# martellab-sri/ModalTune

Hardware: AMD Instinct MI355X
Metric: slides/sec (train step) at 10k patches x 1536-d (higher is better)
Workload: dtype f16; 1 GPU; Prov-GigaPath ModalAdapter train step, 10000 patches x 1536-d, 6 pathways -> 64 gene tokens + 1 task token, 3 task passes, fp16 operands / fp32 accumulate, 1 slide per GPU per step, task passes as two concurrent groups (B = 2 | 1 on two HIP streams), train mode: Dropout(0.25) on the embedded input and both backbone branches, DropPath(0..0.1) per layer and on the Extractor FFN (Philox masks regener; patches=10000, parallelism=dp1, dropout=True

## Files before the change

include/modaltune_hip.h:

```cpp
#ifndef MODALTUNE_HIP_H
#define MODALTUNE_HIP_H

#include <stdint.h>

#ifdef __cplusplus
extern "C" {
#endif

typedef void* mt_stream_t;
typedef uint16_t mt_half;

typedef enum {
  MT_OK = 0,
  MT_ERR_BAD_ARG = -1,
  MT_ERR_LAUNCH = -2,
  MT_ERR_UNSUPPORTED = -3
} MtStatus;

typedef struct { int seg_rows, seg_stride, row0; } MtRowMap;

typedef struct {
  float eps;
  const int* live;
  int live_rows;
  float* partials;
  long partials_elems;
  int grid_wgs;
} MtLaunchOpts;

int mt_version(void);
const char* mt_status_string(int status);
const char* mt_build_id(void);

enum { MT_EPI_BIAS = 0,
       MT_EPI_BIAS_RESID = 1,
       MT_EPI_INJECT = 2,
       MT_EPI_POSEMB = 3,
       MT_EPI_QKV_HM = 4 };
enum { MT_OUT_F16 = 0, MT_OUT_F32 = 1 };

typedef struct {
  const unsigned* rng;
  unsigned site;
  float p;
  unsigned path_site;
  float path_p;
  int rows_per_pass;
} MtDropout;
int mt_rng_advance(unsigned* rng, mt_stream_t stream);
int mt_dropout_f32(const float* x, long ldx, const MtRowMap* xmap, float* y, int M, int D, const MtDropout* drop,
                   mt_stream_t stream);
int mt_droppath_rows_f32(float* x, int M, int D, const MtDropout* drop, mt_stream_t stream);

#define MT_LIVE_SITES_MAX 64
int mt_droppath_live(const unsigned* path_sites, const float* path_ps, int n, int B, const unsigned* rng, int* table,
                     mt_stream_t stream);

typedef struct {
  const float* bias;
  const float* resid;
  long ldr;
  MtRowMap rmap;
  const float* colscale;
  const float* pos_table;
  const int* pos_row;
  const int* pos_col;
  MtDropout drop;
} MtGemmEpilogue;

int mt_gemm_nt_f16(const mt_half* A, long lda, const MtRowMap* amap, const mt_half* W, int M, int N, int K,
                   int epilogue, const MtGemmEpilogue* epi, void* C, long ldc, const MtRowMap* cmap, int out_dtype,
                   const MtLaunchOpts* opt, mt_stream_t stream);

int mt_gemm_tn_f16(const mt_half* A, long lda, const MtRowMap* amap, const mt_half* B, long ldb, const MtRowMap* bmap,
                   int M, int N1, int N2, float* C, long ldc, float* colsum, const MtLaunchOpts* opt, mt_stream_t stream);

int mt_colsum_f16(const mt_half* A, long lda, const MtRowMap* amap, int M, int N, float* out, const MtLaunchOpts* opt,
                  mt_stream_t stream);

enum { MT_ACT_NONE = 0, MT_ACT_RELU = 1, MT_ACT_GELU = 2, MT_ACT_ELU = 3 };
// ... 249 lines not shown
```

modaltune_amd/_lib.py:

```python
from __future__ import annotations

import ctypes as C
import os

_HERE = os.path.dirname(os.path.abspath(__file__))
LIB_PATH = os.environ.get("MODALTUNE_HIP_LIB", os.path.join(_HERE, "_C", "libmodaltune_hip.so"))

P, I, L, F, D = C.c_void_p, C.c_int, C.c_long, C.c_float, C.c_double


class MtRowMap(C.Structure):
    _fields_ = [("seg_rows", I), ("seg_stride", I), ("row0", I)]


class MtDropout(C.Structure):
    _fields_ = [("rng", P), ("site", C.c_uint), ("p", F), ("path_site", C.c_uint), ("path_p", F), ("rows_per_pass", I)]


class MtGemmEpilogue(C.Structure):
    _fields_ = [("bias", P), ("resid", P), ("ldr", L), ("rmap", MtRowMap), ("colscale", P),
                ("pos_table", P), ("pos_row", P), ("pos_col", P), ("drop", MtDropout)]


class MtLaunchOpts(C.Structure):
    _fields_ = [("eps", F), ("live", P), ("live_rows", I), ("partials", P), ("partials_elems", L), ("grid_wgs", I)]


MT_SGEMM_MAX = 3


class MtSgemm(C.Structure):
    _fields_ = [("A", P), ("as0", L), ("as1", L), ("a_bs", L), ("B", P), ("bs0", L), ("bs1", L), ("b_bs", L),
                ("bias", P), ("bias_on_m", I), ("C", P), ("cs0", L), ("cs1", L), ("c_bs", L),
                ("M", I), ("N", I), ("K", I), ("batch", I), ("act", I), ("accumulate", I),
                ("rowsum", P), ("pre_out", P), ("resid", P), ("c_drop", MtDropout),
                ("a_aux", P), ("a_act", I), ("a_drop", MtDropout), ("resid_scale", F), ("a_ld", I)]


MT_MAX_BRANCHES = 8


class MtDilatedPlan(C.Structure):
    _fields_ = [("nbranch", I), ("N", I), ("B", I), ("seg", I * MT_MAX_BRANCHES), ("ratio", I * MT_MAX_BRANCHES),
                ("nseg", I * MT_MAX_BRANCHES), ("n", I * MT_MAX_BRANCHES), ("qlimit", I * MT_MAX_BRANCHES)]


class MtDensePlan(C.Structure):
    _fields_ = [("N", I), ("B", I), ("H", I), ("dist", P), ("nslope", P)]


class MtLongNetLayerWeights(C.Structure):
    _fields_ = [(n, P) for n in ("ln1_w", "ln1_b", "inner_ln_w", "inner_ln_b", "ln2_w", "ln2_b", "ffn_ln_w", "ffn_ln_b", "b_qkv", "b_out",
                                 "b_fc1", "b_fc2", "w_qkv", "w_out", "w_fc1", "w_fc2", "wt_qkv", "wt_out", "wt_fc1", "wt_fc2")]


class MtLongNetLayerBuffers(C.Structure):
    _fields_ = [(n, P) for n in ("hin", "hmid", "qkv", "o_br", "lse_br", "lse_tot", "a1", "st1", "stin", "st2", "stf", "u16", "br16", "t16",
                                 "dh", "dy16", "dh16", "dt16", "da1", "dmixed", "dqkv16", "delta", "attn_ws", "live_attn", "live_ffn")]


class MtVitBlockWeights(C.Structure):
    _fields_ = [(n, P) for n in ("n1_w", "n1_b", "n2_w", "n2_b")] + [("n1_eps", F), ("n2_eps", F)] + \
               [(n, P) for n in ("b_qkv", "b_proj", "b_fc1", "b_fc2", "w_qkv", "w_proj", "w_fc1", "w_fc2", "wt_qkv", "wt_proj", "wt_fc1", "wt_fc2")]


class MtVitBlockBuffers(C.Structure):
    _fields_ = [(n, P) for n in ("hin", "hmid", "qkv", "o16", "lse", "a1", "st1", "st2", "u16", "br16", "t16", "dh", "dy16", "dh16", "dt16",
                                 "da1", "dqkv16", "delta")]


RM = C.POINTER(MtRowMap)
DR = C.POINTER(MtDropout)
EP = C.POINTER(MtGemmEpilogue)
PL = C.POINTER(MtDilatedPlan)
DP = C.POINTER(MtDensePlan)
OP = C.POINTER(MtLaunchOpts)

SIGNATURES = {
# ... 139 lines not shown
```

modaltune_amd/csrc/attn.hip:

```cpp
#include "attn_common.h"

namespace {

template <bool LIVE>
__global__ __launch_bounds__(256) void dilated_attn_fwd_kernel(const h16* __restrict__ qkv, Plan p, h16* __restrict__ o_br,
                                                               float* __restrict__ lse_br) {
  __shared__ __attribute__((aligned(16))) h16 smem[4 * IMG_HALVES];
  h16* const Ks = smem;
  h16* const Vs = smem + 2 * IMG_HALVES;
  const int tid = threadIdx.x, lane = tid & 63, wave = tid >> 6;
  const int hh = lane >> 5, l31 = lane & 31;
  const WorkItem w = decode(p, blockIdx.x);
  const Seq sq = make_seq(p, w);
  const long M = (long)p.B * p.N;
  const int nv = __builtin_amdgcn_readfirstlane(sq.nvalid());
  const int nvq = min(nv, p.qlimit[w.br]);
  if (w.qt * 128 >= nvq || (LIVE && pass_dead(p, w.b))) return;

  {
    const int buf = tid >> 7, row = (tid >> 1) & 63, which = 6 + (tid & 1);
    const h16x8 one = {(h16)1.f, 0, 0, 0, (h16)1.f, 0, 0, 0}, zero = {0, 0, 0, 0, 0, 0, 0, 0};
    *reinterpret_cast<h16x8*>(&Vs[buf * IMG_HALVES + img_off(row, which)]) = which == 6 ? one : zero;
  }

  const int iq = w.qt * 128 + wave * 32 + l31;
  const bool qvalid = sq.valid(iq) && iq < nvq;
  const long qrow = sq.row_clamped(iq);
  h16x8 qf[3];
#pragma unroll
  for (int ks = 0; ks < 3; ++ks)
    qf[ks] = sel8(qvalid, ldg8(hm_ptr(qkv, M, w.h, qrow) + ks * 16 + hh * 8));

  const int ntile = (sq.n + 63) / 64;
  const int nproc = (nv + 63) >> 6;
  const int row_bytes = sq.dr * HD * 2;
  const long valid_bytes = (long)(nv - 1) * row_bytes + HD * 2;
  const long tile_bytes = 64L * row_bytes;
  const h16* const kseq = hm_ptr(qkv, M, H + w.h, sq.row(0));
  const h16* const vseq = hm_ptr(qkv, M, 2 * H + w.h, sq.row(0));
  const DmaLane dl(tid, row_bytes);
  auto dma = [&](int t) {
    dma_tile(Ks + (t & 1) * IMG_HALVES, tile_rsrc(kseq, t * tile_bytes, valid_bytes), dl);
    dma_tile(Vs + (t & 1) * IMG_HALVES, tile_rsrc(vseq, t * tile_bytes, valid_bytes), dl);
  };
  const int grp = lane >> 4, li = lane & 15, tq = li >> 2, tp = li & 3;
  int krd[3];
#pragma unroll
  for (int ks = 0; ks < 3; ++ks) krd[ks] = img_off(l31, 2 * ks + hh);
  const int vc = 2 * (grp & 1) + (tp >> 1), vo = 4 * (tp & 1);
  const int va0 = img_off(4 * hh + tq, vc) + vo, va1 = img_off(4 * hh + tq, vc + 4) + vo;
  const int vb0 = img_off(4 * hh + tq + 8, vc) + vo, vb1 = img_off(4 * hh + tq + 8, vc + 4) + vo;

  auto qk = [&](const h16* Kb, f32x16 (&s)[2], const f32x16& init) {
#pragma unroll
    for (int sub = 0; sub < 2; ++sub) {
#pragma unroll
      for (int ks = 0; ks < 3; ++ks) {
        const h16x8 kf = *reinterpret_cast<const h16x8*>(&Kb[sub * 32 * IMG_ROW + krd[ks]]);
        s[sub] = __builtin_amdgcn_mfma_f32_32x32x16_f16(kf, qf[ks], ks == 0 ? init : s[sub], 0, 0, 0);
      }
    }
  };

  f32x16 o0, o1;
#pragma unroll
  for (int i = 0; i < 16; ++i) { o0[i] = 0.f; o1[i] = 0.f; }

  dma(0);
  dma_wait_all();
  __syncthreads();
  float m2;
  f32x16 minit;
  {
    f32x16 s0[2], zero;
#pragma unroll
    for (int i = 0; i < 16; ++i) zero[i] = 0.f;
    qk(Ks, s0, zero);
    float mx = NEG_BIG;
#pragma unroll
    for (int sub = 0; sub < 2; ++sub)
#pragma unroll
      for (int i = 0; i < 16; ++i) {
        const int kidx = sub * 32 + (i & 3) + 8 * (i >> 2) + 4 * hh;
        mx = fmaxf(mx, kidx < sq.n ? s0[sub][i] : NEG_BIG);
      }
    m2 = max_halves(mx);
#pragma unroll
    for (int i = 0; i < 16; ++i) minit[i] = -m2;
  }

  auto tile = [&](int t, auto tail_tag) {
    constexpr bool TAIL = decltype(tail_tag)::value;
    const int kb = t * 64;
    const h16* Kb = Ks + (t & 1) * IMG_HALVES;
    const h16* Vb = Vs + (t & 1) * IMG_HALVES;
    if (t + 1 < nproc) dma(t + 1);
    f32x16 s_cur[2];
    qk(Kb, s_cur, minit);
    float mx = NEG_BIG;
#pragma unroll
    for (int sub = 0; sub < 2; ++sub)
#pragma unroll
      for (int i = 0; i < 16; ++i) {
        if (TAIL) {
          const int kidx = kb + sub * 32 + (i & 3) + 8 * (i >> 2) + 4 * hh;
          if (kidx >= sq.n) s_cur[sub][i] = NEG_BIG;
        }
        mx = fmaxf(mx, s_cur[sub][i]);
      }
    mx = max_halves(mx);
    if (__any(mx > RESCALE_LOG2)) {
      const float up = fmaxf(mx, 0.f);
      const float alpha = __builtin_amdgcn_exp2f(-up);
#pragma unroll
      for (int i = 0; i < 16; ++i) { o0[i] *= alpha; o1[i] *= alpha; s_cur[0][i] -= up; s_cur[1][i] -= up; }
      m2 += up;
#pragma unroll
      for (int i = 0; i < 16; ++i) minit[i] = -m2;
    }
#pragma unroll
    for (int sub = 0; sub < 2; ++sub)
#pragma unroll
      for (int s2 = 0; s2 < 2; ++s2) {
        h16x8 pf;
#pragma unroll
        for (int e = 0; e < 8; e += 2) {
          const f32x2 a = pk_exp2((f32x2){s_cur[sub][8 * s2 + e], s_cur[sub][8 * s2 + e + 1]});
          pf[e] = (h16)a[0]; pf[e + 1] = (h16)a[1];
        }
        const h16* vblk = Vb + (sub * 32 + s2 * 16) * IMG_ROW;
        const h16x8 v0 = cat8(lds_tr4(vblk + va0), lds_tr4(vblk + vb0));
        const h16x8 v1 = cat8(lds_tr4(vblk + va1), lds_tr4(vblk + vb1));
        o0 = __builtin_amdgcn_mfma_f32_32x32x16_f16(v0, pf, o0, 0, 0, 0);
        o1 = __builtin_amdgcn_mfma_f32_32x32x16_f16(v1, pf, o1, 0, 0, 0);
      }
    dma_wait_all();
    __syncthreads();
  };
  const bool tail_last = nproc == ntile && (sq.n & 63);
  const int nplain = tail_last ? nproc - 1 : nproc;
  for (int t = 0; t < nplain; ++t) tile(t, std::false_type{});
  if (tail_last) tile(nproc - 1, std::true_type{});
  const int rest = sq.n - nproc * 64;
  if (rest > 0) {
    if (__any(-m2 > RESCALE_LOG2)) {
      const float up = fmaxf(-m2, 0.f);
      const float alpha = __builtin_amdgcn_exp2f(-up);
#pragma unroll
      for (int i = 0; i < 16; ++i) { o0[i] *= alpha; o1[i] *= alpha; }
      m2 += up;
    }
    o1[8] += (float)rest * __builtin_amdgcn_exp2f(-m2);
  }

  if (qvalid) {
    const float l = o1[8];
    const float inv = 1.0f / l;
    h16* orow = o_br + ((long)w.br * M + qrow) * DM + w.h * HD;
#pragma unroll
    for (int gq = 0; gq < 4; ++gq) {
      h16x4 v = {(h16)(o0[4 * gq] * inv), (h16)(o0[4 * gq + 1] * inv), (h16)(o0[4 * gq + 2] * inv), (h16)(o0[4 * gq + 3] * inv)};
      *reinterpret_cast<h16x4*>(orow + 8 * gq + 4 * hh) = v;
    }
#pragma unroll
    for (int gq = 0; gq < 2; ++gq) {
      h16x4 v = {(h16)(o1[4 * gq] * inv), (h16)(o1[4 * gq + 1] * inv), (h16)(o1[4 * gq + 2] * inv), (h16)(o1[4 * gq + 3] * inv)};
      *reinterpret_cast<h16x4*>(orow + 32 + 8 * gq + 4 * hh) = v;
    }
    if (hh == 0) lse_br[((long)w.br * M + qrow) * H + w.h] = (m2 + __log2f(l)) * LN2;
  }
}

struct MixGeom {
  int grp[MT_MAX_BRANCHES];
  MT_DEVINL MixGeom(const Plan& p, int h) {
#pragma unroll
    for (int b = 0; b < MT_MAX_BRANCHES; ++b) grp[b] = b < p.nbranch ? h / (H / p.ratio[b]) : -1;
  }
};
MT_DEVINL void seg_split(const Plan& p, int b, int pos, int& j, int& loc) {
  const int sg = p.seg[b];
  if (sg >= p.N) { j = 0; loc = pos; return; }
  j = (int)((float)pos * p.inv_seg[b]);
  loc = pos - j * sg;
  if (loc < 0) { loc += sg; --j; }
  if (loc >= sg) { loc -= sg; ++j; }
}
MT_DEVINL int residue(const Plan& p, int b, int pos) {
  int j, loc;
  seg_split(p, b, pos, j, loc);
  const int dr = p.ratio[b];
  return (dr & (dr - 1)) == 0 ? (loc & (dr - 1)) : loc % dr;
}
MT_DEVINL int dense_branch(const Plan& p) {
  int d = 0;
#pragma unroll
  for (int b = 0; b < MT_MAX_BRANCHES; ++b) if (b < p.nbranch && p.ratio[b] == 1) d = b;
  return d;
}
constexpr int MIX_CPL = 24;
struct H24 { h16x8 a, b, c; };
MT_DEVINL H24 ld24(const h16* p) {
  return H24{*reinterpret_cast<const h16x8*>(p), *reinterpret_cast<const h16x8*>(p + 8), *reinterpret_cast<const h16x8*>(p + 16)};
}
MT_DEVINL float h24(const H24& v, int e) { return (float)(e < 8 ? v.a[e & 7] : e < 16 ? v.b[e & 7] : v.c[e & 7]); }
MT_DEVINL float half_sum(float v) {
// ... 98 lines not shown
    for (int b = 0; b < NB; ++b) {
      cov[b] = b < p.nbranch && geo.grp[b] == residue(p, b, pos);
      const int sb = cov[b] ? b : db;
      lse[b] = lse_br[((long)sb * M + m) * H + h];
      ob[b] = ld24(o_br + ((long)sb * M + m) * DM + c0);
    }
    float v[MIX_CPL];
#pragma unroll
    for (int e = 0; e < MIX_CPL; ++e) v[e] = 0.f;
#pragma unroll
    for (int b = 0; b < NB; ++b) {
      const float wgt = cov[b] ? __expf(lse[b] - tot) : 0.f;
#pragma unroll
      for (int e = 0; e < MIX_CPL; ++e) v[e] = fmaf(wgt, cov[b] ? h24(ob[b], e) : 0.f, v[e]);
    }
    float g[MIX_CPL], xh[MIX_CPL];
    float s1 = 0.f, s2 = 0.f;
#pragma unroll
    for (int i = 0; i < MIX_CPL; ++i) {
      xh[i] = (v[i] - mean) * rstd;
      g[i] = h24(dyv, i) * w[i];
      s1 += g[i]; s2 = fmaf(g[i], xh[i], s2);
    }
    const float c1 = half_sum(s1) * (1.0f / DM), c2 = half_sum(s2) * (1.0f / DM);
    float dm[MIX_CPL];
    h16* dst = dmixed + ((long)h * M + m) * HD + (c0 - h * HD);
#pragma unroll
    for (int k = 0; k < 3; ++k) {
      h16x8 o;
#pragma unroll
      for (int e = 0; e < 8; ++e) {
        const int i = 8 * k + e;
        o[e] = (h16)(rstd * (g[i] - c1 - xh[i] * c2));
        dm[i] = (float)o[e];
      }
      if (live) *reinterpret_cast<h16x8*>(dst + 8 * k) = o;
    }
#pragma unroll
    for (int b = 0; b < NB; ++b) {
      float d = 0.f;
#pragma unroll
      for (int e = 0; e < MIX_CPL; ++e) d = fmaf(dm[e], h24(ob[b], e), d);
      d += __shfl_xor(d, 1, 64);
      if (live && (l5 & 1) == 0 && cov[b]) delta_br[((long)b * M + m) * H + h] = d;
    }
  }
}


}

extern "C" int mt_dilated_attn_fwd(const mt_half* qkv, const MtDilatedPlan* plan, mt_half* o_br, float* lse_br, const MtLaunchOpts* opt,
                                   mt_stream_t stream) {
  if (int rc = mt_opts_check(opt, MT_OPT_LIVE)) return rc;
  if (!qkv || !o_br || !lse_br || !plan_ok(plan)) return MT_ERR_BAD_ARG;
  const Plan p = make_plan(plan, 128, mt_opt_live(opt));
  const int nblk = p.blk_off[p.nbranch];
  if (p.live) hipLaunchKernelGGL(dilated_attn_fwd_kernel<true>, dim3(nblk), dim3(256), 0, (hipStream_t)stream, (const h16*)qkv, p,
                     (h16*)o_br, lse_br);
  else hipLaunchKernelGGL(dilated_attn_fwd_kernel<false>, dim3(nblk), dim3(256), 0, (hipStream_t)stream, (const h16*)qkv, p,
                     (h16*)o_br, lse_br);
  MT_CHECK_LAUNCH();
  return MT_OK;
}

constexpr int MIX_CUS = 256, MIX_FWD_WG_PER_CU = 3, MIX_BWD_WG_PER_CU = 2;
static dim3 mix_grid(long M, int grid_wgs, int wg_per_cu) {
  return dim3((int)min((M + 7) / 8, (long)(grid_wgs > 0 ? grid_wgs : wg_per_cu * MIX_CUS)));
}

extern "C" int mt_dilated_mix_ln_fwd(const mt_half* o_br, const float* lse_br, const MtDilatedPlan* plan,
                                     const float* ln_w, const float* ln_b, mt_half* y, float* stats, float* lse_tot,
                                     const MtLaunchOpts* opt, mt_stream_t stream) {
  if (int rc = mt_opts_check(opt, MT_OPT_LIVE | MT_OPT_GRID)) return rc;
  if (!o_br || !lse_br || !ln_w || !ln_b || !y || !stats || !lse_tot || !plan_ok(plan)) return MT_ERR_BAD_ARG;
  const Plan p = make_plan(plan, 128, mt_opt_live(opt));
  const long M = (long)p.B * p.N;
  const dim3 grid = mix_grid(M, opt ? opt->grid_wgs : 0, MIX_FWD_WG_PER_CU);
  if (p.nbranch <= 5)
    hipLaunchKernelGGL(mix_ln_fwd_kernel<5>, grid, dim3(256), 0, (hipStream_t)stream, (const h16*)o_br, lse_br, p, ln_w, ln_b,
                       (h16*)y, stats, lse_tot);
  else
    hipLaunchKernelGGL(mix_ln_fwd_kernel<MT_MAX_BRANCHES>, grid, dim3(256), 0, (hipStream_t)stream, (const h16*)o_br, lse_br, p,
                       ln_w, ln_b, (h16*)y, stats, lse_tot);
  MT_CHECK_LAUNCH();
  return MT_OK;
}

extern "C" int mt_dilated_mix_ln_bwd(const mt_half* dy, const mt_half* o_br, const float* lse_br, const float* lse_tot,
                                     const MtDilatedPlan* plan, const float* ln_w, const float* stats, mt_half* dmixed,
                                     float* delta_br, const MtLaunchOpts* opt, mt_stream_t stream) {
  if (int rc = mt_opts_check(opt, MT_OPT_LIVE | MT_OPT_GRID)) return rc;
  if (!dy || !o_br || !lse_br || !lse_tot || !ln_w || !stats || !dmixed || !delta_br || !plan_ok(plan)) return MT_ERR_BAD_ARG;
  const Plan p = make_plan(plan, 128, mt_opt_live(opt));
  const long M = (long)p.B * p.N;
  const dim3 grid = mix_grid(M, opt ? opt->grid_wgs : 0, MIX_BWD_WG_PER_CU);
  if (p.nbranch <= 5)
    hipLaunchKernelGGL(mix_ln_bwd_kernel<5>, grid, dim3(256), 0, (hipStream_t)stream, (const h16*)dy, (const h16*)o_br, lse_br,
                       lse_tot, p, ln_w, stats, (h16*)dmixed, delta_br);
  else
    hipLaunchKernelGGL(mix_ln_bwd_kernel<MT_MAX_BRANCHES>, grid, dim3(256), 0, (hipStream_t)stream, (const h16*)dy,
                       (const h16*)o_br, lse_br, lse_tot, p, ln_w, stats, (h16*)dmixed, delta_br);
  MT_CHECK_LAUNCH();
  return MT_OK;
}

extern "C" long mt_dilated_attn_bwd_workspace_bytes(const MtDilatedPlan* plan) {
  if (!plan_ok(plan)) return MT_ERR_BAD_ARG;
  const Plan p = make_plan(plan, 128);
  return p.ws_off[p.nbranch] * (long)sizeof(h16);
}

namespace {
int attn_bwd(const mt_half* qkv, const mt_half* dmixed, const float* lse_tot, const float* delta_br, const MtDilatedPlan* plan,
// ... 30 lines not shown
```

modaltune_amd/csrc/common.h:

```cpp
#pragma once
#include <hip/hip_runtime.h>
#include <stdint.h>

#include "../../include/modaltune_hip.h"

typedef _Float16 h16;
typedef _Float16 h16x2 __attribute__((ext_vector_type(2)));
typedef _Float16 h16x4 __attribute__((ext_vector_type(4)));
typedef _Float16 h16x8 __attribute__((ext_vector_type(8)));
typedef short s16x4 __attribute__((ext_vector_type(4)));
typedef float f32x2 __attribute__((ext_vector_type(2)));
typedef float f32x4 __attribute__((ext_vector_type(4)));
typedef float f32x16 __attribute__((ext_vector_type(16)));

#define MT_WAVE 64
#define MT_DEVINL __device__ __forceinline__
MT_DEVINL float lds_f32(const float* p) { return *reinterpret_cast<const volatile float*>(p); }
MT_DEVINL f32x4 lds_f32x4_by_dword(const float* p) {
  const volatile float* q = reinterpret_cast<const volatile float*>(p);
  return (f32x4){q[0], q[1], q[2], q[3]};
}
#define MT_LDS_DRAIN_V1(a) asm volatile("s_waitcnt lgkmcnt(0)" : "+v"(a) : : "memory")
#define MT_LDS_DRAIN_V2(a, b) asm volatile("s_waitcnt lgkmcnt(0)" : "+v"(a), "+v"(b) : : "memory")
#define MT_LDS_DRAIN_V3(a, b, c) asm volatile("s_waitcnt lgkmcnt(0)" : "+v"(a), "+v"(b), "+v"(c) : : "memory")
// ... 83 lines not shown
MT_DEVINL f32x4 drop_elem4(const DropArgs& d, uint64_t idx4, float pf) {
  f32x4 s = {pf, pf, pf, pf};
  if (d.p > 0.f) {
    uint32_t r[4];
    philox4x32_7((uint32_t)idx4, (uint32_t)(idx4 >> 32), d.site, d.rng[2], d.rng[0], d.rng[1], r);
    const uint32_t thr = drop_threshold(d.p);
    const float keep = pf / (1.f - d.p);
#pragma unroll
    for (int e = 0; e < 4; ++e) s[e] = r[e] >= thr ? keep : 0.f;
  }
  return s;
}
MT_DEVINL f32x4 drop_apply4(f32x4 v, f32x4 s) {
#pragma unroll
  for (int e = 0; e < 4; ++e) v[e] = s[e] != 0.f ? v[e] * s[e] : 0.f;
  return v;
}
struct RowRange { int first, end; };
MT_DEVINL RowRange live_rows_of(const int* live, int rows_per_pass, int M) {
  RowRange r = {0, M};
  if (live) {
    r.first = (int)min((long)max(live[0], 0) * rows_per_pass, (long)M);
    r.end = max(r.first, (int)min((long)max(live[1], 0) * rows_per_pass, (long)M));
  }
  return r;
}
MT_DEVINL f32x4 drop_scale4(const DropArgs& d, uint64_t idx4, int m) {
  return drop_elem4(d, idx4, drop_path_factor(d, m / d.rows_per_pass));
}

MT_DEVINL bool drop_keep1(const DropArgs& d, uint32_t site, uint64_t idx) {
  uint32_t r[4];
  philox4x32_7((uint32_t)(idx >> 2), (uint32_t)(idx >> 34), site, d.rng[2], d.rng[0], d.rng[1], r);
  return r[idx & 3] >= drop_threshold(d.p);
}

MT_DEVINL uint32_t drop_keep4(const DropArgs& d, uint64_t idx4, uint32_t thr) {
  uint32_t r[4];
  philox4x32_7((uint32_t)idx4, (uint32_t)(idx4 >> 32), d.site, d.rng[2], d.rng[0], d.rng[1], r);
  return (r[0] >= thr ? 1u : 0u) | (r[1] >= thr ? 2u : 0u) | (r[2] >= thr ? 4u : 0u) | (r[3] >= thr ? 8u : 0u);
}

MT_DEVINL h16x8 ldg8(const h16* p) { return *reinterpret_cast<const h16x8*>(p); }
MT_DEVINL void stg8(h16* p, h16x8 v) { *reinterpret_cast<h16x8*>(p) = v; }

#define MT_CHECK_LAUNCH()                                   \
  do {                                                      \
    hipError_t e__ = hipGetLastError();                     \
    if (e__ != hipSuccess) return MT_ERR_LAUNCH;            \
  } while (0)

static inline int cdiv(long a, long b) { return (int)((a + b - 1) / b); }

enum { MT_OPT_EPS = 1, MT_OPT_LIVE = 2, MT_OPT_PARTIALS = 4, MT_OPT_GRID = 8 };
static inline int mt_opts_check(const MtLaunchOpts* o, int allowed) {
  if (!o) return MT_OK;
  const int set = (o->eps != 0.f ? MT_OPT_EPS : 0) | (o->live || o->live_rows ? MT_OPT_LIVE : 0) |
                  (o->partials || o->partials_elems ? MT_OPT_PARTIALS : 0) | (o->grid_wgs ? MT_OPT_GRID : 0);
  if (set & ~allowed) return MT_ERR_UNSUPPORTED;
  if (!(o->eps >= 0.f) || o->live_rows < 0 || o->partials_elems < 0 || o->grid_wgs < 0) return MT_ERR_BAD_ARG;
  if (o->partials_elems && !o->partials) return MT_ERR_BAD_ARG;
  return MT_OK;
}
static inline float mt_opt_eps(const MtLaunchOpts* o) { return o && o->eps != 0.f ? o->eps : 1e-5f; }
static inline const int* mt_opt_live(const MtLaunchOpts* o) { return o ? o->live : nullptr; }
static inline float* mt_opt_partials(const MtLaunchOpts* o) { return o ? o->partials : nullptr; }

int mt_det_reduce_launch(const float* partials, int nparts, int rows, int cols, long part_stride, float* dst, long ldd, hipStream_t s);
```

modaltune_amd/csrc/optim.hip:

```cpp
#include "common.h"

namespace {

__global__ __launch_bounds__(256) void distill_loss_kernel(const float* __restrict__ logits, const float* __restrict__ target, int R, int O,
                                                           float loss_scale_host, const float* __restrict__ scale_dev,
                                                           float* __restrict__ loss, float* __restrict__ dlogits) {
  const float loss_scale = loss_scale_host * (scale_dev ? *scale_dev : 1.0f);
  __shared__ float red[256];
  __shared__ float bc[4];
  const int tid = threadIdx.x;
  auto block_sum = [&](float v) {
    red[tid] = v; __syncthreads();
    for (int s = 128; s > 0; s >>= 1) { if (tid < s) red[tid] += red[tid + s]; __syncthreads(); }
    const float r = red[0]; __syncthreads(); return r;
  };
  auto block_max = [&](float v) {
    red[tid] = v; __syncthreads();
    for (int s = 128; s > 0; s >>= 1) { if (tid < s) red[tid] = fmaxf(red[tid], red[tid + s]); __syncthreads(); }
    const float r = red[0]; __syncthreads(); return r;
  };
  float total = 0.f;
  for (int r = 0; r < R; ++r) {
    const float* lg = logits + (long)r * O;
    const float* tg = target + (long)r * O;
// ... 318 lines not shown
                     found_inf, out);
  MT_CHECK_LAUNCH();
  return MT_OK;
}

extern "C" int mt_absmax_scale(const float* x, long n, float target, float* s, mt_stream_t stream) {
  if (!x || !s || n <= 0 || !(target > 0.f)) return MT_ERR_BAD_ARG;
  hipLaunchKernelGGL(absmax_scale_kernel, dim3(1), dim3(256), 0, (hipStream_t)stream, x, n, target, s);
  MT_CHECK_LAUNCH();
  return MT_OK;
}

extern "C" int mt_axpy_dev(const float* a, const float* b, const float* alpha, float* y, long n, mt_stream_t stream) {
  if (!b || !alpha || !y || n <= 0) return MT_ERR_BAD_ARG;
  const int grid = (int)((n + 1023) / 1024 > 4096 ? 4096 : (n + 1023) / 1024);
  hipLaunchKernelGGL(axpy_dev_kernel, dim3(grid), dim3(256), 0, (hipStream_t)stream, a, b, alpha, y, n);
  MT_CHECK_LAUNCH();
  return MT_OK;
}

extern "C" int mt_mfma_probe(float* sink, int workgroups, int iters, mt_stream_t stream) {
  if (!sink || workgroups < 1 || iters < 1) return MT_ERR_BAD_ARG;
  hipLaunchKernelGGL(mfma_probe_kernel, dim3(workgroups), dim3(256), 0, (hipStream_t)stream, sink, iters);
  MT_CHECK_LAUNCH();
  return MT_OK;
}

extern "C" int mt_coords_to_grid(const float* coords, int L, float tile, int ngrids, int* prow, int* pcol, int* err,
                                 mt_stream_t stream) {
  if (!coords || !prow || !pcol || L < 1 || !(tile > 0.f) || ngrids < 1) return MT_ERR_BAD_ARG;
  hipLaunchKernelGGL(coords_to_grid_kernel, dim3((L + 255) / 256), dim3(256), 0, (hipStream_t)stream, coords, L, tile, ngrids, prow,
                     pcol, err);
  MT_CHECK_LAUNCH();
  return MT_OK;
}

extern "C" int mt_scatter_rows_f32(const float* src, const int* src_idx, const int* idx, float* dst, int M, int D, int accumulate,
                                   mt_stream_t stream) {
  if (!src || !idx || !dst || M < 1 || D < 1) return MT_ERR_BAD_ARG;
  const long n = (long)M * D;
  const int grid = (int)((n + 255) / 256 > 8192 ? 8192 : (n + 255) / 256);
  hipLaunchKernelGGL(scatter_rows_kernel, dim3(grid), dim3(256), 0, (hipStream_t)stream, src, src_idx, idx, dst, M, D, accumulate);
  MT_CHECK_LAUNCH();
  return MT_OK;
}

extern "C" int mt_row_absmax_f32(const float* x, float* out, int M, int D, mt_stream_t stream) {
  if (!x || !out || M < 1 || D < 1) return MT_ERR_BAD_ARG;
  hipLaunchKernelGGL(row_absmax_kernel, dim3((M + 3) / 4 > 4096 ? 4096 : (M + 3) / 4), dim3(256), 0, (hipStream_t)stream, x, out, M, D);
  MT_CHECK_LAUNCH();
  return MT_OK;
}

extern "C" int mt_version(void) { return 320; }

extern "C" const char* mt_status_string(int status) {
  switch (status) {
    case MT_OK: return "ok";
    case MT_ERR_BAD_ARG: return "bad argument (shape / alignment / null pointer)";
    case MT_ERR_LAUNCH: return "kernel launch failed";
    case MT_ERR_UNSUPPORTED: return "unsupported configuration";
    default: return "unknown status";
  }
}
```

modaltune_amd/ops.py:

```python
from __future__ import annotations

import ctypes as C
import os
from typing import Optional, Sequence

import torch

from . import _lib
from ._lib import MtLongNetLayerBuffers, MtLongNetLayerWeights, MtVitBlockBuffers, MtVitBlockWeights
from ._lib import MT_SGEMM_MAX, MtDensePlan, MtDilatedPlan, MtDropout, MtGemmEpilogue, MtLaunchOpts, MtRowMap, MtSgemm, check, rowmap

F16, F32 = 0, 1
EPI_BIAS, EPI_BIAS_RESID, EPI_INJECT, EPI_POSEMB, EPI_QKV_HM = 0, 1, 2, 3, 4
ACT_NONE, ACT_RELU, ACT_GELU, ACT_ELU = 0, 1, 2, 3


def _p(t: Optional[torch.Tensor]):
    return None if t is None else t.data_ptr()


_raw_stream = getattr(torch._C, "_cuda_getCurrentRawStream", None)
_raw_device = getattr(torch._C, "_cuda_getDevice", None)


def _s():
    if _raw_stream is not None and _raw_device is not None:
        return _raw_stream(_raw_device())
    return torch.cuda.current_stream().cuda_stream


def _dt(t: torch.Tensor) -> int:
    if t.dtype == torch.float16:
        return F16
    if t.dtype == torch.float32:
        return F32
    raise TypeError(f"unsupported dtype {t.dtype}")


def _rm(m):
    return None if m is None else C.byref(m)


def _need(t, dtype, name):
    if t.dtype != dtype or not t.is_cuda or not t.is_contiguous():
        raise TypeError(f"{name}: expected contiguous cuda {dtype}, got {t.dtype} cuda={t.is_cuda} contig={t.is_contiguous()}")


def make_plan(branches, N: int, B: int, qlimit=None) -> MtDilatedPlan:
    p = MtDilatedPlan()
    p.nbranch, p.N, p.B = len(branches), N, B
    for i, b in enumerate(branches):
        p.seg[i], p.ratio[i], p.nseg[i], p.n[i] = b.seg, b.ratio, b.nseg, b.n
        p.qlimit[i] = 0 if qlimit is None else int(qlimit[i])
    return p


def dropout_spec(rng, site=0, p=0.0, path_site=0, path_p=0.0, rows_per_pass=1) -> MtDropout:
    d = MtDropout()
    d.rng, d.site, d.p, d.path_site, d.path_p, d.rows_per_pass = rng.data_ptr(), site, p, path_site, path_p, rows_per_pass
    return d


def _dr(d):
    return C.byref(d) if d is not None else None


def _opts(what="", *, eps=1e-5, live=None, live_rows=0, det=None, grid_wgs=0):
    if eps == 1e-5 and live is None and det is None and not grid_wgs:
        return None
    o = MtLaunchOpts()
    if eps != 1e-5:
        if not eps > 0:
            check(-1, what)
        o.eps = float(eps)
    if live is not None:
        o.live, o.live_rows = live.data_ptr(), int(live_rows)
    if det is not None:
        _need(det, torch.float32, "det")
        if det.numel() == 0:
            check(-1, what)
        o.partials, o.partials_elems = det.data_ptr(), det.numel()
    o.grid_wgs = int(grid_wgs)
    return C.byref(o)


def gemm_nt(A, W, out, M, N, K, *, lda=None, amap=None, ldc=None, cmap=None, epilogue=EPI_BIAS, bias=None, resid=None,
            ldr=0, rmap=None, colscale=None, pos_table=None, pos_row=None, pos_col=None, drop=None, live=None, live_rows=0):
    epi = MtGemmEpilogue()
    if drop is not None:
        epi.drop = drop
    epi.bias, epi.resid, epi.ldr = (bias.data_ptr() if bias is not None else None,
                                    resid.data_ptr() if resid is not None else None, ldr)
    if rmap is not None:
        epi.rmap = rmap
    epi.colscale = colscale.data_ptr() if colscale is not None else None
    epi.pos_table = pos_table.data_ptr() if pos_table is not None else None
    epi.pos_row = pos_row.data_ptr() if pos_row is not None else None
    epi.pos_col = pos_col.data_ptr() if pos_col is not None else None
    check(_lib.load().mt_gemm_nt_f16(_p(A), lda if lda is not None else K, _rm(amap), _p(W), M, N, K, epilogue,
                                     C.byref(epi), _p(out), ldc if ldc is not None else N, _rm(cmap), _dt(out),
                                     _opts(live=live, live_rows=live_rows), _s()), "gemm_nt")


def det_elems(name: str, *shape) -> int:
    n = getattr(_lib.load(), f"mt_{name}_det_elems")(*shape)
    if n < 0:
        check(int(n), f"{name}_det_elems{shape}")
    return int(n)


def gemm_tn(A, B, out, M, N1, N2, *, lda=None, amap=None, ldb=None, bmap=None, ldc=None, colsum=None, det=None):
    what = "gemm_tn" if det is None else "gemm_tn_det"
    check(_lib.load().mt_gemm_tn_f16(_p(A), lda if lda is not None else N1, _rm(amap), _p(B), ldb if ldb is not None else N2,
                                     _rm(bmap), M, N1, N2, _p(out), ldc if ldc is not None else N2, _p(colsum), _opts(what, det=det), _s()),
          what)


def colsum(A, out, M, N, *, lda=None, amap=None, det=None):
    what = "colsum" if det is None else "colsum_det"
    check(_lib.load().mt_colsum_f16(_p(A), lda if lda is not None else N, _rm(amap), M, N, _p(out), _opts(what, det=det), _s()), what)


def sgemm_problem(A, a_str, B, b_str, Cm, c_str, M, N, K, *, bias=None, bias_on_m=False, act=ACT_NONE, accumulate=False,
                  batch=1, a_bs=0, b_bs=0, c_bs=0, rowsum=None, pre_out=None, resid=None, c_drop=None, a_aux=None,
                  a_act=ACT_NONE, a_drop=None, resid_scale=1.0, a_ld=0) -> MtSgemm:
    q = MtSgemm()
    q.A, q.as0, q.as1, q.a_bs = _p(A), a_str[0], a_str[1], a_bs
    q.B, q.bs0, q.bs1, q.b_bs = _p(B), b_str[0], b_str[1], b_bs
    q.bias, q.bias_on_m = _p(bias), int(bias_on_m)
    q.C, q.cs0, q.cs1, q.c_bs = _p(Cm), c_str[0], c_str[1], c_bs
    q.M, q.N, q.K, q.batch, q.act, q.accumulate = M, N, K, batch, act, int(accumulate)
    q.rowsum, q.pre_out, q.resid = _p(rowsum), _p(pre_out), _p(resid)
    if c_drop is not None:
        q.c_drop = c_drop
    q.a_aux, q.a_act = _p(a_aux), a_act
    if a_drop is not None:
        q.a_drop = a_drop
    q.resid_scale, q.a_ld = float(resid_scale), int(a_ld)
    return q


def sgemm_multi(problems):
    for i in range(0, len(problems), MT_SGEMM_MAX):
        chunk = problems[i:i + MT_SGEMM_MAX]
        arr = (MtSgemm * len(chunk))(*chunk)
        check(_lib.load().mt_sgemm_multi(arr, len(chunk), _s()), "sgemm_multi")


def sgemm(A, a_str, B, b_str, Cm, c_str, M, N, K, **k):
    sgemm_multi([sgemm_problem(A, a_str, B, b_str, Cm, c_str, M, N, K, **k)])


def layernorm_fwd(x, w, b, y, stats, M, D, *, ldx=None, xmap=None, ldy=None, ymap=None, gelu_in=False, add_rows=None,
                  add_period=0, eps=1e-5, live=None, live_rows=0):
    check(_lib.load().mt_layernorm_fwd(_p(x), ldx if ldx is not None else D, _rm(xmap), _dt(x), int(gelu_in), _p(w), _p(b),
                                       _p(add_rows), add_period, _p(y), ldy if ldy is not None else D, _rm(ymap), _dt(y),
                                       _p(stats), M, D, _opts("layernorm_fwd", eps=eps, live=live, live_rows=live_rows), _s()),
          "layernorm_fwd")


def add_layernorm_fwd(x, branch, w, b, h, y, stats, M, D, drop=None, eps=1e-5):
    check(_lib.load().mt_add_layernorm_fwd(_p(x), _p(branch), _dr(drop), _p(w), _p(b), _p(h), _p(y), _p(stats), M, D,
                                           _opts("add_layernorm_fwd", eps=eps), _s()), "add_layernorm_fwd")


def layernorm_bwd(dy, x, w, stats, dx, M, D, *, lddy=None, dymap=None, ldx=None, xmap=None, lddx=None, dxmap=None,
                  gelu_in=False, accumulate=False, dw=None, db=None, dx16=None, dx16_drop=None, det=None, live=None, live_rows=0):
    if live is not None and dw is not None:
        raise ValueError("layernorm_bwd: a live table goes with a frozen norm (dw / db of a trainable one sum over every row)")
    if dw is None:
        det = None
    what = "layernorm_bwd" if det is None else "layernorm_bwd_det"
    check(_lib.load().mt_layernorm_bwd(_p(dy), lddy if lddy is not None else D, _rm(dymap), _dt(dy), _p(x), ldx if ldx is not None else D,
                                       _rm(xmap), _dt(x), int(gelu_in), _p(w), _p(stats), _p(dx), lddx if lddx is not None else D,
                                       _rm(dxmap), _dt(dx), int(accumulate), _p(dw), _p(db), _p(dx16), _dr(dx16_drop), M, D,
                                       _opts(what, live=live, live_rows=live_rows, det=det), _s()), what)


LIVE_SITES_MAX = 64


def droppath_live(path_sites, path_ps, B, rng, table):
    n = len(path_sites)
    check(_lib.load().mt_droppath_live((C.c_uint * n)(*path_sites), (C.c_float * n)(*path_ps), n, B, _p(rng), _p(table), _s()),
          "droppath_live")


def dilated_attn_fwd(qkv, plan, o_br, lse_br, live=None):
    check(_lib.load().mt_dilated_attn_fwd(_p(qkv), C.byref(plan), _p(o_br), _p(lse_br), _opts(live=live), _s()), "dilated_attn_fwd")


def dilated_mix_ln_fwd(o_br, lse_br, plan, ln_w, ln_b, y, stats, lse_tot, live=None, grid_wgs=0):
    check(_lib.load().mt_dilated_mix_ln_fwd(_p(o_br), _p(lse_br), C.byref(plan), _p(ln_w), _p(ln_b), _p(y), _p(stats), _p(lse_tot),
                                            _opts(live=live, grid_wgs=grid_wgs), _s()), "dilated_mix_ln_fwd")


def dilated_mix_ln_bwd(dy, o_br, lse_br, lse_tot, plan, ln_w, stats, dmixed, delta_br, live=None, grid_wgs=0):
    check(_lib.load().mt_dilated_mix_ln_bwd(_p(dy), _p(o_br), _p(lse_br), _p(lse_tot), C.byref(plan), _p(ln_w), _p(stats), _p(dmixed),
                                            _p(delta_br), _opts(live=live, grid_wgs=grid_wgs), _s()), "dilated_mix_ln_bwd")


def dilated_mix_ln_fwd_grid(o_br, lse_br, plan, ln_w, ln_b, y, stats, lse_tot, grid_wgs=0):
    dilated_mix_ln_fwd(o_br, lse_br, plan, ln_w, ln_b, y, stats, lse_tot, grid_wgs=grid_wgs)


def dilated_mix_ln_bwd_grid(dy, o_br, lse_br, lse_tot, plan, ln_w, stats, dmixed, delta_br, grid_wgs=0):
    dilated_mix_ln_bwd(dy, o_br, lse_br, lse_tot, plan, ln_w, stats, dmixed, delta_br, grid_wgs=grid_wgs)


def dilated_attn_bwd_workspace_bytes(plan) -> int:
    n = _lib.load().mt_dilated_attn_bwd_workspace_bytes(C.byref(plan))
    if n < 0:
        check(int(n), "dilated_attn_bwd_workspace_bytes")
    return int(n)


ATTN_BWD_KV, ATTN_BWD_Q, ATTN_BWD_COMBINE, ATTN_BWD_ALL = 1, 2, 4, 7


def _dilated_attn_bwd_phase(qkv, dmixed, lse_tot, delta_br, plan, workspace, dqkv16, phases):
    check(_lib.load().mt_dilated_attn_bwd(_p(qkv), _p(dmixed), _p(lse_tot), _p(delta_br), C.byref(plan), _p(workspace),
                                          _p(dqkv16), phases, _s()), "dilated_attn_bwd")


def dilated_attn_bwd_phases(qkv, dmixed, lse_tot, delta_br, plan, workspace, dqkv16, phases):
    _dilated_attn_bwd_phase(qkv, dmixed, lse_tot, delta_br, plan, workspace, dqkv16, phases)


def dilated_attn_bwd_inplace_phases(qkv, dmixed, lse_tot, delta_br, plan, workspace, dqkv16, phases=ATTN_BWD_ALL, live=None):
    check(_lib.load().mt_dilated_attn_bwd_inplace(_p(qkv), _p(dmixed), _p(lse_tot), _p(delta_br), C.byref(plan), _p(workspace), _p(dqkv16),
                                                  phases, _opts(live=live), _s()), "dilated_attn_bwd_inplace")


def dilated_attn_bwd(qkv, dmixed, lse_tot, delta_br, plan, workspace, dqkv16):
    if TIMER is None:
        return _dilated_attn_bwd_phase(qkv, dmixed, lse_tot, delta_br, plan, workspace, dqkv16, ATTN_BWD_ALL)
    for key, ph in (("dilated_attn_bwd_kv", ATTN_BWD_KV), ("dilated_attn_bwd_q", ATTN_BWD_Q), ("dilated_attn_bwd_combine", ATTN_BWD_COMBINE)):
        _bracket(key, _dilated_attn_bwd_phase, qkv, dmixed, lse_tot, delta_br, plan, workspace, dqkv16, ph)


DENSE_QK_SCALE_LOG2 = 0.125 * 1.4426950408889634
DENSE_BWD_DELTA, DENSE_BWD_KV, DENSE_BWD_Q, DENSE_BWD_ALL = 1, 2, 4, 7
# ... 448 lines not shown
```

Before: 25.81 slides/s.

## Skip per-tile online-softmax max tracking in attention forward, recompute on overflow

The dilated attention forward kernel now runs every key tile using only the first-tile max as its fixed softmax reference, dropping the per-tile max reduction and rescale check. If the accumulated denominator overflows or becomes non-finite, the workgroup discards its accumulators, reloads tile 0 and reruns all tiles with full max tracking, optionally counting these fallbacks in a stats counter. This removes a cross-lane max and branch per tile on the common path. In exchange, rows that overflow pay for a second full pass, an extra workgroup barrier is added, and fp16 precision may be lost when later scores greatly exceed the first tile's max without actually overflowing.

```diff
diff --git a/include/modaltune_hip.h b/include/modaltune_hip.h
--- a/include/modaltune_hip.h
+++ b/include/modaltune_hip.h
@@ -26,6 +26,7 @@
   float* partials;
   long partials_elems;
   int grid_wgs;
+  int* stats;
 } MtLaunchOpts;
 
 int mt_version(void);
diff --git a/modaltune_amd/_lib.py b/modaltune_amd/_lib.py
--- a/modaltune_amd/_lib.py
+++ b/modaltune_amd/_lib.py
@@ -23,7 +23,7 @@
 
 
 class MtLaunchOpts(C.Structure):
-    _fields_ = [("eps", F), ("live", P), ("live_rows", I), ("partials", P), ("partials_elems", L), ("grid_wgs", I)]
+    _fields_ = [("eps", F), ("live", P), ("live_rows", I), ("partials", P), ("partials_elems", L), ("grid_wgs", I), ("stats", P)]
 
 
 MT_SGEMM_MAX = 3
diff --git a/modaltune_amd/csrc/attn.hip b/modaltune_amd/csrc/attn.hip
--- a/modaltune_amd/csrc/attn.hip
+++ b/modaltune_amd/csrc/attn.hip
@@ -2,9 +2,9 @@
 
 namespace {
 
-template <bool LIVE>
+template <bool LIVE, bool TRACK_ONLY = false>
 __global__ __launch_bounds__(256) void dilated_attn_fwd_kernel(const h16* __restrict__ qkv, Plan p, h16* __restrict__ o_br,
-                                                               float* __restrict__ lse_br) {
+                                                               float* __restrict__ lse_br, int* __restrict__ stats) {
   __shared__ __attribute__((aligned(16))) h16 smem[4 * IMG_HALVES];
   h16* const Ks = smem;
   h16* const Vs = smem + 2 * IMG_HALVES;
@@ -71,7 +71,7 @@
   __syncthreads();
   float m2;
   f32x16 minit;
-  {
+  auto tile0_reference = [&](int n_keys) {
     f32x16 s0[2], zero;
 #pragma unroll
     for (int i = 0; i < 16; ++i) zero[i] = 0.f;
@@ -82,41 +82,46 @@
 #pragma unroll
       for (int i = 0; i < 16; ++i) {
         const int kidx = sub * 32 + (i & 3) + 8 * (i >> 2) + 4 * hh;
-        mx = fmaxf(mx, kidx < sq.n ? s0[sub][i] : NEG_BIG);
+        mx = fmaxf(mx, kidx < n_keys ? s0[sub][i] : NEG_BIG);
       }
     m2 = max_halves(mx);
 #pragma unroll
     for (int i = 0; i < 16; ++i) minit[i] = -m2;
-  }
-
-  auto tile = [&](int t, auto tail_tag) {
-    constexpr bool TAIL = decltype(tail_tag)::value;
+  };
+  tile0_reference(sq.n);
+
+  auto tile = [&](int t, auto tail_tag, auto track_tag) {
+    constexpr bool TAIL = decltype(tail_tag)::value, TRACK = decltype(track_tag)::value;
     const int kb = t * 64;
     const h16* Kb = Ks + (t & 1) * IMG_HALVES;
     const h16* Vb = Vs + (t & 1) * IMG_HALVES;
     if (t + 1 < nproc) dma(t + 1);
     f32x16 s_cur[2];
     qk(Kb, s_cur, minit);
-    float mx = NEG_BIG;
-#pragma unroll
-    for (int sub = 0; sub < 2; ++sub)
-#pragma unroll
-      for (int i = 0; i < 16; ++i) {
-        if (TAIL) {
-          const int kidx = kb + sub * 32 + (i & 3) + 8 * (i >> 2) + 4 * hh;
-          if (kidx >= sq.n) s_cur[sub][i] = NEG_BIG;
+    if (TAIL || TRACK) {
+      float mx = NEG_BIG;
+#pragma unroll
+      for (int sub = 0; sub < 2; ++sub)
+#pragma unroll
+        for (int i = 0; i < 16; ++i) {
+          if (TAIL) {
+            const int kidx = kb + sub * 32 + (i & 3) + 8 * (i >> 2) + 4 * hh;
+            if (kidx >= sq.n) s_cur[sub][i] = NEG_BIG;
+          }
+          if (TRACK) mx = fmaxf(mx, s_cur[sub][i]);
         }
-        mx = fmaxf(mx, s_cur[sub][i]);
-      }
-    mx = max_halves(mx);
-    if (__any(mx > RESCALE_LOG2)) {
-      const float up = fmaxf(mx, 0.f);
-      const float alpha = __builtin_amdgcn_exp2f(-up);
-#pragma unroll
-      for (int i = 0; i < 16; ++i) { o0[i] *= alpha; o1[i] *= alpha; s_cur[0][i] -= up; s_cur[1][i] -= up; }
-      m2 += up;
-#pragma unroll
-      for (int i = 0; i < 16; ++i) minit[i] = -m2;
+      if (TRACK) {
+        mx = max_halves(mx);
+        if (__any(mx > RESCALE_LOG2)) {
+          const float up = fmaxf(mx, 0.f);
+          const float alpha = __builtin_amdgcn_exp2f(-up);
+#pragma unroll
+          for (int i = 0; i < 16; ++i) { o0[i] *= alpha; o1[i] *= alpha; s_cur[0][i] -= up; s_cur[1][i] -= up; }
+          m2 += up;
+#pragma unroll
+          for (int i = 0; i < 16; ++i) minit[i] = -m2;
+        }
+      }
     }
 #pragma unroll
     for (int sub = 0; sub < 2; ++sub)
@@ -139,19 +144,42 @@
   };
   const bool tail_last = nproc == ntile && (sq.n & 63);
   const int nplain = tail_last ? nproc - 1 : nproc;
-  for (int t = 0; t < nplain; ++t) tile(t, std::false_type{});
-  if (tail_last) tile(nproc - 1, std::true_type{});
   const int rest = sq.n - nproc * 64;
-  if (rest > 0) {
-    if (__any(-m2 > RESCALE_LOG2)) {
-      const float up = fmaxf(-m2, 0.f);
-      const float alpha = __builtin_amdgcn_exp2f(-up);
-#pragma unroll
-      for (int i = 0; i < 16; ++i) { o0[i] *= alpha; o1[i] *= alpha; }
-      m2 += up;
-    }
-    o1[8] += (float)rest * __builtin_amdgcn_exp2f(-m2);
-  }
+  auto all_tiles = [&](auto track_tag) {
+    for (int t = 0; t < nplain; ++t) tile(t, std::false_type{}, track_tag);
+    if (tail_last) tile(nproc - 1, std::true_type{}, track_tag);
+    if (rest > 0) {
+      if (__any(-m2 > RESCALE_LOG2)) {
+        const float up = fmaxf(-m2, 0.f);
+        const float alpha = __builtin_amdgcn_exp2f(-up);
+#pragma unroll
+        for (int i = 0; i < 16; ++i) { o0[i] *= alpha; o1[i] *= alpha; }
+        m2 += up;
+      }
+      o1[8] += (float)rest * __builtin_amdgcn_exp2f(-m2);
+    }
+  };
+  bool tracked = TRACK_ONLY;
+  if (!TRACK_ONLY) {
+    all_tiles(std::false_type{});
+    int* const flag = reinterpret_cast<int*>(&Ks[img_off(0, 6)]);
+    const bool inexact = __any(!(fabsf(o1[8]) <= 3.0e38f));
+    if (lane == 0) flag[wave] = inexact;
+    __syncthreads();
+    tracked = __builtin_amdgcn_readfirstlane(flag[0] | flag[1] | flag[2] | flag[3]) != 0;
+    if (tracked) {
+      if (stats && tid == 0) atomicAdd(stats, 1);
+#pragma unroll
+      for (int i = 0; i < 16; ++i) { o0[i] = 0.f; o1[i] = 0.f; }
+      dma(0);
+      dma_wait_all();
+      __syncthreads();
+      int n_again = sq.n;
+      asm volatile("" : "+s"(n_again));
+      tile0_reference(n_again);
+    }
+  }
+  if (tracked) all_tiles(std::true_type{});
 
   if (qvalid) {
     const float l = o1[8];
@@ -356,14 +384,17 @@
 
 extern "C" int mt_dilated_attn_fwd(const mt_half* qkv, const MtDilatedPlan* plan, mt_half* o_br, float* lse_br, const MtLaunchOpts* opt,
                                    mt_stream_t stream) {
-  if (int rc = mt_opts_check(opt, MT_OPT_LIVE)) return rc;
+  if (int rc = mt_opts_check(opt, MT_OPT_LIVE | MT_OPT_STATS)) return rc;
   if (!qkv || !o_br || !lse_br || !plan_ok(plan)) return MT_ERR_BAD_ARG;
+  static const char* force = getenv("MT_ATTN_FWD_TRACK");
+  const bool track_only = force && force[0] == '1';
   const Plan p = make_plan(plan, 128, mt_opt_live(opt));
   const int nblk = p.blk_off[p.nbranch];
-  if (p.live) hipLaunchKernelGGL(dilated_attn_fwd_kernel<true>, dim3(nblk), dim3(256), 0, (hipStream_t)stream, (const h16*)qkv, p,
-                     (h16*)o_br, lse_br);
-  else hipLaunchKernelGGL(dilated_attn_fwd_kernel<false>, dim3(nblk), dim3(256), 0, (hipStream_t)stream, (const h16*)qkv, p,
-                     (h16*)o_br, lse_br);
+  auto launch = [&](auto kernel) {
+    hipLaunchKernelGGL(kernel, dim3(nblk), dim3(256), 0, (hipStream_t)stream, (const h16*)qkv, p, (h16*)o_br, lse_br, mt_opt_stats(opt));
+  };
+  if (p.live) track_only ? launch(dilated_attn_fwd_kernel<true, true>) : launch(dilated_attn_fwd_kernel<true>);
+  else track_only ? launch(dilated_attn_fwd_kernel<false, true>) : launch(dilated_attn_fwd_kernel<false>);
   MT_CHECK_LAUNCH();
   return MT_OK;
 }
diff --git a/modaltune_amd/csrc/common.h b/modaltune_amd/csrc/common.h
--- a/modaltune_amd/csrc/common.h
+++ b/modaltune_amd/csrc/common.h
@@ -159,11 +159,11 @@
 
 static inline int cdiv(long a, long b) { return (int)((a + b - 1) / b); }
 
-enum { MT_OPT_EPS = 1, MT_OPT_LIVE = 2, MT_OPT_PARTIALS = 4, MT_OPT_GRID = 8 };
+enum { MT_OPT_EPS = 1, MT_OPT_LIVE = 2, MT_OPT_PARTIALS = 4, MT_OPT_GRID = 8, MT_OPT_STATS = 16 };
 static inline int mt_opts_check(const MtLaunchOpts* o, int allowed) {
   if (!o) return MT_OK;
   const int set = (o->eps != 0.f ? MT_OPT_EPS : 0) | (o->live || o->live_rows ? MT_OPT_LIVE : 0) |
-                  (o->partials || o->partials_elems ? MT_OPT_PARTIALS : 0) | (o->grid_wgs ? MT_OPT_GRID : 0);
+                  (o->partials || o->partials_elems ? MT_OPT_PARTIALS : 0) | (o->grid_wgs ? MT_OPT_GRID : 0) | (o->stats ? MT_OPT_STATS : 0);
   if (set & ~allowed) return MT_ERR_UNSUPPORTED;
   if (!(o->eps >= 0.f) || o->live_rows < 0 || o->partials_elems < 0 || o->grid_wgs < 0) return MT_ERR_BAD_ARG;
   if (o->partials_elems && !o->partials) return MT_ERR_BAD_ARG;
@@ -172,5 +172,6 @@
 static inline float mt_opt_eps(const MtLaunchOpts* o) { return o && o->eps != 0.f ? o->eps : 1e-5f; }
 static inline const int* mt_opt_live(const MtLaunchOpts* o) { return o ? o->live : nullptr; }
 static inline float* mt_opt_partials(const MtLaunchOpts* o) { return o ? o->partials : nullptr; }
+static inline int* mt_opt_stats(const MtLaunchOpts* o) { return o ? o->stats : nullptr; }
 
 int mt_det_reduce_launch(const float* partials, int nparts, int rows, int cols, long part_stride, float* dst, long ldd, hipStream_t s);
diff --git a/modaltune_amd/csrc/optim.hip b/modaltune_amd/csrc/optim.hip
--- a/modaltune_amd/csrc/optim.hip
+++ b/modaltune_amd/csrc/optim.hip
@@ -394,7 +394,7 @@
   return MT_OK;
 }
 
-extern "C" int mt_version(void) { return 320; }
+extern "C" int mt_version(void) { return 330; }
 
 extern "C" const char* mt_status_string(int status) {
   switch (status) {
diff --git a/modaltune_amd/ops.py b/modaltune_amd/ops.py
--- a/modaltune_amd/ops.py
+++ b/modaltune_amd/ops.py
@@ -65,8 +65,8 @@
     return C.byref(d) if d is not None else None
 
 
-def _opts(what="", *, eps=1e-5, live=None, live_rows=0, det=None, grid_wgs=0):
-    if eps == 1e-5 and live is None and det is None and not grid_wgs:
+def _opts(what="", *, eps=1e-5, live=None, live_rows=0, det=None, grid_wgs=0, stats=None):
+    if eps == 1e-5 and live is None and det is None and not grid_wgs and stats is None:
         return None
     o = MtLaunchOpts()
     if eps != 1e-5:
@@ -81,6 +81,9 @@
             check(-1, what)
         o.partials, o.partials_elems = det.data_ptr(), det.numel()
     o.grid_wgs = int(grid_wgs)
+    if stats is not None:
+        _need(stats, torch.int32, "stats")
+        o.stats = stats.data_ptr()
     return C.byref(o)
 
 
@@ -186,8 +189,9 @@
           "droppath_live")
 
 
-def dilated_attn_fwd(qkv, plan, o_br, lse_br, live=None):
-    check(_lib.load().mt_dilated_attn_fwd(_p(qkv), C.byref(plan), _p(o_br), _p(lse_br), _opts(live=live), _s()), "dilated_attn_fwd")
+def dilated_attn_fwd(qkv, plan, o_br, lse_br, live=None, stats=None):
+    check(_lib.load().mt_dilated_attn_fwd(_p(qkv), C.byref(plan), _p(o_br), _p(lse_br), _opts(live=live, stats=stats), _s()),
+          "dilated_attn_fwd")
 
 
 def dilated_mix_ln_fwd(o_br, lse_br, plan, ln_w, ln_b, y, stats, lse_tot, live=None, grid_wgs=0):
```

Result: no change. 25.91 slides/s (median of 6 runs) (+0.4%).
